# JuliaHealth/Thunderbolt.jl

Hardware: AMD Instinct MI355X
Metric: element-integrations/sec + DoF-updates/sec, 10M-hex Q1 monodomain (higher is better)
Workload: dtype f64

## Files before the change

### thunderbolt.jl_amd/csrc/tb_internal.h

```cpp
#pragma once
#include <cstdio>
#include <cstdlib>
#include <ctime>
#include <hip/hip_runtime.h>

#include <cstdint>
#include <cstdio>
#include <cstdlib>
#include <memory>
#include <string>
#include <vector>

#include "tbhip.h"
#include "tb_planners.hpp"

namespace tb {

void set_error(const char *fmt, ...);
#ifdef TB_ABLATION
inline const char *tune_env(const char *name) { return getenv(name); }
#else
inline const char *tune_env(const char *) { return nullptr; }
#endif
void set_last_kernel(const char *fmt, ...);
// ... 68 lines not shown

struct PatchPlan : plan::PatchHost {
    int version = 0;
    int64_t *d_elem_ptr = nullptr;
    int64_t *d_row_ptr = nullptr;
    int32_t *d_elem_cell = nullptr;
    uint16_t *d_elem_lrow = nullptr;
    int32_t *d_row_dof = nullptr;
};

struct PatchMatPlan {
    int version = 0;
    int max_lds_entries = 0;
    RowDesc *d_row_desc = nullptr;
    uint16_t *d_elem_rowoff = nullptr;
    uint8_t *d_colpos8 = nullptr;
    uint16_t *d_colpos16 = nullptr;
};

struct PatchFusedPlan {
    int version = 0;
    int max_lds_entries = 0, max_nodes = 0;
    int64_t nsig = 0;
    int64_t *d_node_ptr = nullptr;
    int32_t *d_pnode = nullptr;
    uint16_t *d_elem_ln = nullptr;
    uint32_t *d_elem_sig = nullptr;
    uint8_t *d_sigtab = nullptr;
    RowDesc *d_row_desc = nullptr;
    uint32_t *d_hdr = nullptr;
    double *d_pcoord = nullptr;
    uint8_t *d_rec = nullptr;
    int rec_stride = 0, rec_rm = 0, rec_nm = 0, rec_ne = 0;
};

struct VecPatchPlan {
    bool halo = false;
    int64_t n_patches = 0, total_elems = 0, total_nodes = 0;
    int max_nodes = 0, max_elems = 0;
    uint32_t *d_hdr = nullptr;
    uint16_t *d_elem_ln = nullptr;
    int32_t *d_elem_cell = nullptr;
    double *d_pcoord = nullptr;
    int32_t *d_pdof = nullptr;
};

constexpr int RED_SLOTS = 64, RED_STRIDE = 16, RED_GROUP = RED_SLOTS * RED_STRIDE;

}

struct tb_pattern;
struct tb_device {
    int id = 0;
    hipStream_t stream = nullptr;
    bool own_stream = true;
    int n_cu = 0;
    size_t hbm_bytes = 0;
    std::string name;
    tb::Status *d_status = nullptr;
    tb::Status *h_status = nullptr;
    bool defer_status = false;
    void *d_scratch = nullptr;
    size_t scratch_bytes = 0;
    double *d_slots = nullptr;
    double *d_readback = nullptr;
    double *d_tslot = nullptr;
// ... 259 lines not shown
```

### thunderbolt.jl_amd/csrc/tb_patch_fused.hip

```cpp
#include <hip/hip_runtime.h>

#include <algorithm>
#include <cstdio>
#include <cstring>
#include <vector>

#include "tb_elem.hpp"
#include "tb_forms.hpp"
#include "tb_hex8_sumfac.hpp"
#include "tb_internal.h"

namespace tb {
using namespace tbk;

struct FusedView {
    const int64_t *elem_ptr, *row_ptr, *node_ptr;
    const int32_t *elem_cell;
    const uint16_t *elem_ln;
    const uint32_t *elem_sig;
    const uint8_t *sigtab;
    const int32_t *pnode;
    const RowDesc *row_desc;
    int kcap, max_rows, max_nodes;
#ifdef TB_ABLATION
    long long *prof;
#endif
};

template <bool WK, bool WM, bool FK, bool FM, bool DIAG = false, bool ISO = false, class Meta>
__device__ __forceinline__ void hex8_instance(const double (&x)[8][3], Meta &&meta, int64_t cell, const FormArgs &faK,
                                              const FormArgs &faM, double *accK, double *accM, Status *st, const int32_t *elem_cell, int64_t e)
{
    double G[8][6], dq[8];
    if constexpr (FK) {
        const double *gp = faK.gtab + cell * 56;
#pragma unroll
        for (int q = 0; q < 8; ++q) {
#pragma unroll
            for (int k = 0; k < 6; ++k) G[q][k] = gp[7 * q + k];
            dq[q] = gp[7 * q + 6];
        }
    } else {
        auto Dq = [&](int, double(&D)[6]) { D[0] = faK.D[0]; D[1] = faK.D[1]; D[2] = faK.D[2]; D[3] = faK.D[4]; D[4] = faK.D[5]; D[5] = faK.D[8]; };
#ifdef TB_ABLATION
        if (faK.debug & 4) {
#pragma unroll
            for (int q = 0; q < 8; ++q) { dq[q] = x[q][0] + x[q][1] + x[q][2]; for (int k = 0; k < 6; ++k) G[q][k] = dq[q]; }
        } else
#endif
        if (!hex8_sf_geometry<WK, false, DIAG, ISO>(x, Dq, G, dq, ISO ? faK.iso_scale : -0.25)) { st->neg_detj = 1; st->cell = elem_cell ? elem_cell[e] : -1; }
    }
    Hex8SFK c;
    if constexpr (WK) hex8_sf_contract(G, c);
    uint4 cp[4];
    uint32_t ro[8];
    meta(cp, ro);
    bool own[8];
#pragma unroll
    for (int i = 0; i < 8; ++i) own[i] = ro[i] != 0xFFFFFFFFu;
#ifdef TB_ABLATION
    if (faK.debug & 1) {
#pragma unroll
        for (int i = 1; i < 8; ++i) own[i] = false;
        own[0] = own[0] && (G[0][0] + dq[0] == 1.2345);
    }
#endif
    auto pos = [&](int i, int j) -> uint32_t {
        const uint4 &c4 = cp[i >> 1];
        const uint32_t w = (i & 1) ? (j < 4 ? c4.z : c4.w) : (j < 4 ? c4.x : c4.y);
        return (w >> (8 * (j & 3))) & 0xffu;
    };
    if constexpr (WK) {
#pragma unroll
        for (int i = 0; i < 8; ++i)
#pragma unroll
            for (int j = i; j < 8; ++j) {
                const double v = hex8_sf_entry(c, i, j);
                if (own[i]) unsafeAtomicAdd(accK + (ro[i] + pos(i, j)), v);
                if (j > i && own[j]) unsafeAtomicAdd(accK + (ro[j] + pos(j, i)), v);
            }
    }
    if constexpr (WM) {
        if constexpr (FM) {
            double rn[8];
#pragma unroll
            for (int a = 0; a < 8; ++a) rn[a] = faM.field[cell * 8 + a];
#pragma unroll
            for (int q = 0; q < 8; ++q) {
                double r = 0.0;
#pragma unroll
                for (int a = 0; a < 8; ++a) r += Hex8<2>::N(q, a) * rn[a];
                dq[q] *= r;
            }
        } else {
#pragma unroll
            for (int q = 0; q < 8; ++q) dq[q] *= faM.rho;
        }
        double Z[3][3][3];
        hex8_sf_mass(dq, Z);
#pragma unroll
        for (int i = 0; i < 8; ++i)
            if (own[i]) {
#pragma unroll
                for (int j = 0; j < 8; ++j) unsafeAtomicAdd(accM + (ro[i] + pos(i, j)), Z[SF::ty(i, j, 0)][SF::ty(i, j, 1)][SF::ty(i, j, 2)]);
            }
    }
}

__global__ void __launch_bounds__(256)
k_tabulate_g_hex8(MeshView m, const double *__restrict__ dtab, double *__restrict__ gtab, Status *st)
{
    const int64_t cell = (int64_t)blockIdx.x * blockDim.x + threadIdx.x;
    if (cell >= m.n_cells) return;
    double x[8][3];
#pragma unroll
    for (int a = 0; a < 8; ++a) {
        const double *px = m.xyz + 3 * (int64_t)m.conn[cell * 8 + a];
        x[a][0] = px[0]; x[a][1] = px[1]; x[a][2] = px[2];
    }
    double G[8][6], dq[8];
    auto Dq = [&](int q, double(&D)[6]) {
        const double *dp = dtab + (cell * 8 + q) * 6;
#pragma unroll
        for (int k = 0; k < 6; ++k) D[k] = dp[k];
    };
    if (!hex8_sf_geometry<true, false>(x, Dq, G, dq)) { st->neg_detj = 1; st->cell = cell; }
    double *gp = gtab + cell * 56;
#pragma unroll
    for (int q = 0; q < 8; ++q) {
#pragma unroll
        for (int k = 0; k < 6; ++k) gp[7 * q + k] = G[q][k];
        gp[7 * q + 6] = dq[q];
    }
}

template <bool WK, bool WM, bool FK, bool FM>
__global__ void __launch_bounds__(256, 2)
// ... 156 lines not shown
    for (int s0 = half; s0 < nrows; s0 += 4 * (T / 32)) {
        uint4 d[4];
#pragma unroll
        for (int u = 0; u < 4; ++u) { const int s = s0 + u * (T / 32); d[u] = ((const uint4 *)desc)[s < nrows ? s : s0]; if (s >= nrows) d[u].w = 0; }
        double vK[4], vM[4];
#pragma unroll
        for (int u = 0; u < 4; ++u) {
            const uint32_t a_ = d[u].z + (hl < d[u].w ? hl : 0);
            if constexpr (WK) vK[u] = accK[a_];
            if constexpr (WM) vM[u] = accM[a_];
        }
#pragma unroll
        for (int u = 0; u < 4; ++u)
            if (hl < d[u].w) {
                const int64_t g0 = (int64_t)(((uint64_t)d[u].y << 32) | d[u].x) + hl;
                if constexpr (WK) nzK[g0] = vK[u];
                if constexpr (WM) nzM[g0] = vM[u];
            }
#pragma unroll
        for (int u = 0; u < 4; ++u)
            for (uint32_t k = hl + 32; k < d[u].w; k += 32) {
                const int64_t g0 = (int64_t)(((uint64_t)d[u].y << 32) | d[u].x) + k;
                if constexpr (WK) nzK[g0] = accK[d[u].z + k];
                if constexpr (WM) nzM[g0] = accM[d[u].z + k];
            }
    }
    TB_ST(5);
#ifdef TB_ABLATION
    if (pv.prof) { __builtin_amdgcn_s_waitcnt(0); TB_ST(6); }
#endif
#undef TB_ST
}

template <bool WK, bool WM, bool DIAG, bool ISO, int RPH, int KOFF = 0, bool WQ = true>
__global__ void __launch_bounds__(256, 2)
k_patch_hex8_record(FormArgs faK, FormArgs faM, const uint8_t *__restrict__ rec, int stride, int nem, int rm, int nm, int kcap, const uint8_t *__restrict__ sigtab, const int32_t *__restrict__ elem_cell, int pf, int prio, int stagger,
                    double *__restrict__ nzK, double *__restrict__ nzM, Status *st
#ifdef TB_ABLATION
                    , long long *prof
#endif
)
{
    extern __shared__ double lds[];
    constexpr int T = 256;
    const int tid = threadIdx.x;
    const int wave_s = __builtin_amdgcn_readfirstlane(threadIdx.x >> 6);
#ifdef TB_ABLATION
#define TB_ST(k) do { if (prof && tid == 0 && (blockIdx.x & 1023) == 7) prof[(blockIdx.x >> 10) * 8 + (k)] = wall_clock64(); } while (0)
#else
#define TB_ST(k) do { } while (0)
#endif
    TB_ST(0);
    bool slot0 = false;
    if (prio >= 2) slot0 = (__builtin_amdgcn_s_getreg((31 << 11) | 6) & 0xfffu) == 0u;
    if (prio == 1 || prio == 2) __builtin_amdgcn_s_setprio(3);
    if (stagger > 0 && blockIdx.x >= 256 && blockIdx.x < 512)
        for (int k = 0; k < stagger; k += 100) __builtin_amdgcn_s_sleep(100);
    const uint8_t *r = rec + (size_t)blockIdx.x * (size_t)stride;
    const uint4 h4 = *(const uint4 *)r;
    const uint32_t hw = h4.x;
    (void)pf;
    uint4 lnv = ((const uint4 *)(r + 16))[tid];
    const uint32_t sig = ((const uint32_t *)(r + 16 + (size_t)nem * 16))[tid];
    const uint8_t *rdp = r + 16 + (size_t)nem * 20;
    const double *pc = (const double *)(rdp + (size_t)rm * 16);
    constexpr int NX = ISO ? 6 : 5;
    uint4 rd = make_uint4(0, 0, 0, 0);
    double xc[NX];
    if (tid < rm) rd = ((const uint4 *)rdp)[tid];
    if constexpr (ISO) {
#pragma unroll
        for (int j = 0; j < 2; ++j)
#pragma unroll
            for (int d = 0; d < 3; ++d) xc[3 * j + d] = tid + j * T < nm ? pc[3 * (tid + j * T) + d] : 0.0;
    } else {
#pragma unroll
        for (int j = 0; j < NX; ++j) xc[j] = tid + j * T < 3 * nm ? pc[tid + j * T] : 0.0;
    }
    const int kblk = KOFF > 0 ? KOFF : kcap;
    double *accK = lds;
    double *accM = lds + (WK && WM ? kblk : 0);
    RowDesc *desc = (RowDesc *)(lds + (WK && WM ? 2 : 1) * kblk);
    double *xs = (double *)(desc + rm);
    {
        double2 *z = (double2 *)lds;
        const int n2 = ((WK && WM ? 2 : 1) * kblk) >> 1;
        for (int k = tid; k < n2; k += T) z[k] = make_double2(0.0, 0.0);
    }
    if (tid < rm) ((uint4 *)desc)[tid] = rd;
    if constexpr (ISO) {
        const double *Li = faK.Linv;
        auto put = [&](int node, double x0, double x1, double x2) {
            xs[3 * node] = Li[0] * x0 + Li[1] * x1 + Li[2] * x2; xs[3 * node + 1] = Li[3] * x0 + Li[4] * x1 + Li[5] * x2; xs[3 * node + 2] = Li[6] * x0 + Li[7] * x1 + Li[8] * x2;
        };
#pragma unroll
        for (int j = 0; j < 2; ++j) if (tid + j * T < nm) put(tid + j * T, xc[3 * j], xc[3 * j + 1], xc[3 * j + 2]);
        for (int k = tid + 2 * T; k < nm; k += T) put(k, pc[3 * k], pc[3 * k + 1], pc[3 * k + 2]);
    } else {
#pragma unroll
        for (int j = 0; j < NX; ++j) if (tid + j * T < 3 * nm) xs[tid + j * T] = xc[j];
        for (int k = tid + NX * T; k < 3 * nm; k += T) xs[k] = pc[k];
    }
    uint4 cp[4];
    {
        const uint4 *cpp = (const uint4 *)(sigtab + (size_t)sig * 64);
#pragma unroll
        for (int k = 0; k < 4; ++k) cp[k] = cpp[k];
    }
    const int nrows = (int)(hw & 0x3ff), ne = (int)(hw >> 21);
    TB_ST(1);
    __syncthreads();
    TB_ST(2);
    if (prio == 1) __builtin_amdgcn_s_setprio(0);
    else if (prio >= 2) { if (!slot0) __builtin_amdgcn_s_setprio(0); else if (prio == 4) __builtin_amdgcn_s_setprio(1); else __builtin_amdgcn_s_setprio(3); }
    for (int ei = tid; ei < ne; ei += T) {
        if (ei >= T) {
            lnv = ((const uint4 *)(r + 16))[ei];
            const uint4 *cpp = (const uint4 *)(sigtab + (size_t)((const uint32_t *)(r + 16 + (size_t)nem * 16))[ei] * 64);
#pragma unroll
            for (int k = 0; k < 4; ++k) cp[k] = cpp[k];
        }
        const uint32_t ln[8] = {lnv.x & 0xffffu, lnv.x >> 16, lnv.y & 0xffffu, lnv.y >> 16, lnv.z & 0xffffu, lnv.z >> 16, lnv.w & 0xffffu, lnv.w >> 16};
        double x[8][3];
#pragma unroll
        for (int a = 0; a < 8; ++a) {
            const double *px = xs + 3 * ln[a];
            x[a][0] = px[0]; x[a][1] = px[1]; x[a][2] = px[2];
        }
        uint32_t ro[8];
#pragma unroll
        for (int i = 0; i < 8; ++i) ro[i] = ln[i] < (uint32_t)nrows ? desc[ln[i]].off : 0xFFFFFFFFu;
        hex8_instance<WK, WM, false, false, DIAG, ISO>(x, [&](uint4(&c4)[4], uint32_t(&r8)[8]) { for (int k = 0; k < 4; ++k) c4[k] = cp[k]; for (int k = 0; k < 8; ++k) r8[k] = ro[k]; }, 0, faK, faM, accK, accM, st,
                                                  elem_cell, (int64_t)h4.y + ei);
    }
    TB_ST(3);
    __syncthreads();
    TB_ST(4);
    if (prio == 1 || prio == 2) __builtin_amdgcn_s_setprio(3);
    const int tidw = (int)__builtin_amdgcn_mbcnt_hi(~0u, __builtin_amdgcn_mbcnt_lo(~0u, 0u)) + 64 * wave_s;
    if constexpr (WQ) {
        const int quarter = tidw >> 4, e2 = (tidw & 15) << 1;
        constexpr int RQ = RPH / 2, RH = RQ / 2;
#pragma unroll
        for (int h = 0; h < 2; ++h) {
            uint4 d[RH];
#pragma unroll
            for (int u = 0; u < RH; ++u) { const int s = quarter + (h * RH + u) * (T / 16); d[u] = ((const uint4 *)desc)[s < nrows ? s : 0]; }
            asm volatile("" ::: "memory");
#pragma unroll
            for (int u = 0; u < RH; ++u) if (quarter + (h * RH + u) * (T / 16) >= nrows) d[u].w = 0;
            double vK[RH][2], vM[RH][2];
#pragma unroll
            for (int u = 0; u < RH; ++u) {
                const uint32_t a_ = d[u].z + ((uint32_t)e2 < d[u].w ? e2 : 0);
                if constexpr (WK) { vK[u][0] = accK[a_]; vK[u][1] = accK[a_ + 1]; }
                if constexpr (WM) { vM[u][0] = accM[a_]; vM[u][1] = accM[a_ + 1]; }
            }
#pragma unroll
            for (int u = 0; u < RH; ++u) {
                const int64_t g0 = (int64_t)(((uint64_t)d[u].y << 32) | d[u].x) + e2;
                if ((uint32_t)e2 + 1 < d[u].w) {
                    if constexpr (WK) *(double2 *)(nzK + g0) = make_double2(vK[u][0], vK[u][1]);
                    if constexpr (WM) *(double2 *)(nzM + g0) = make_double2(vM[u][0], vM[u][1]);
                } else if ((uint32_t)e2 < d[u].w) {
                    if constexpr (WK) nzK[g0] = vK[u][0];
                    if constexpr (WM) nzM[g0] = vM[u][0];
// ... 133 lines not shown
                          (size_t)2 * KOFF * sizeof(double) + (size_t)pr->rec_rm * sizeof(RowDesc) + (size_t)pr->rec_nm * 3 * sizeof(double) <= 80 * 1024;
        const size_t ldsr = (size_t)nreg * (fixm ? KOFF : pv.kcap) * sizeof(double) + (size_t)pr->rec_rm * sizeof(RowDesc) + (size_t)pr->rec_nm * 3 * sizeof(double);
        if (ldsr <= 80 * 1024) {
            constexpr int RPH = 20;
            static const bool iso_on = !(getenv("TB_PATCH_ISO") && atoi(getenv("TB_PATCH_ISO")) == 0);
            bool iso = false;
            FormArgs aMi = aM;
            if (fK && iso_on) {
                const double *D = aK.D;
                double L[3][3] = {{0, 0, 0}, {0, 0, 0}, {0, 0, 0}};
                bool pd = D[1] == D[3] && D[2] == D[6] && D[5] == D[7];
                for (int i = 0; i < 3 && pd; ++i)
                    for (int j = 0; j <= i; ++j) {
                        double sum = D[3 * i + j];
                        for (int k2 = 0; k2 < j; ++k2) sum -= L[i][k2] * L[j][k2];
                        if (i == j) { if (!(sum > 0.0)) { pd = false; break; } L[i][i] = std::sqrt(sum); }
                        else L[i][j] = sum / L[j][j];
                    }
                if (pd) {
                    double Li[3][3] = {{0, 0, 0}, {0, 0, 0}, {0, 0, 0}};
                    for (int i = 0; i < 3; ++i) {
                        Li[i][i] = 1.0 / L[i][i];
                        for (int j = 0; j < i; ++j) { double sum = 0.0; for (int k2 = j; k2 < i; ++k2) sum -= L[i][k2] * Li[k2][j]; Li[i][j] = sum / L[i][i]; }
                    }
                    const double detL = L[0][0] * L[1][1] * L[2][2];
                    for (int i = 0; i < 3; ++i) for (int j = 0; j < 3; ++j) aK.Linv[3 * i + j] = Li[i][j];
                    aK.iso_scale = -0.25 * detL;
                    aMi.rho = aM.rho * detL;
                    iso = true;
                }
            }
            static const size_t lds_pad = tune_env("TB_PATCH_LDS_PAD") ? (size_t)atol(tune_env("TB_PATCH_LDS_PAD")) : 0;
            const size_t ldsr_ = ldsr;
            auto launch_rec = [&](auto k) -> int {
                const size_t ldsr = std::max(ldsr_, lds_pad);
                TB_HIP(hipFuncSetAttribute((const void *)k, hipFuncAttributeMaxDynamicSharedMemorySize, (int)ldsr));
#ifdef TB_ABLATION
                hipLaunchKernelGGL(k, dim3((unsigned)pp->n_patches), dim3(256), ldsr, dev->stream, aK, aMi, (const uint8_t *)pr->d_rec, pr->rec_stride, pr->rec_ne, pr->rec_rm, pr->rec_nm, pv.kcap,
                                   (const uint8_t *)pf->d_sigtab, pp->d_elem_cell, pf_ahead, wave_prio, stagger, d_nzK, d_nzM, dev->d_status, d_prof);
#else
                hipLaunchKernelGGL(k, dim3((unsigned)pp->n_patches), dim3(256), ldsr, dev->stream, aK, aMi, (const uint8_t *)pr->d_rec, pr->rec_stride, pr->rec_ne, pr->rec_rm, pr->rec_nm, pv.kcap,
                                   (const uint8_t *)pf->d_sigtab, pp->d_elem_cell, pf_ahead, wave_prio, stagger, d_nzK, d_nzM, dev->d_status);
#endif
                return TB_OK;
            };
            set_last_kernel("k_patch_hex8_record<%s,%s,RPH%d%s>", fK && fM ? "K+M" : fK ? "K" : "M", !fK ? "-" : iso ? "ISO" : diag ? "DIAG" : "GEN", RPH, fK && fM && fixm ? ",KOFF4096" : "");
            static const bool wq_off = tune_env("TB_PATCH_WQ") && atoi(tune_env("TB_PATCH_WQ")) == 0;
            if (fK && fM && fixm && iso && wq_off) rc = launch_rec(k_patch_hex8_record<true, true, false, true, RPH, KOFF, false>);
            else if (fK && fM && fixm) rc = iso ? launch_rec(k_patch_hex8_record<true, true, false, true, RPH, KOFF>) : diag ? launch_rec(k_patch_hex8_record<true, true, true, false, RPH, KOFF>) : launch_rec(k_patch_hex8_record<true, true, false, false, RPH, KOFF>);
            else if (fK && fM) rc = iso ? launch_rec(k_patch_hex8_record<true, true, false, true, RPH>) : diag ? launch_rec(k_patch_hex8_record<true, true, true, false, RPH>) : launch_rec(k_patch_hex8_record<true, true, false, false, RPH>);
            else if (fK) rc = iso ? launch_rec(k_patch_hex8_record<true, false, false, true, RPH>) : diag ? launch_rec(k_patch_hex8_record<true, false, true, false, RPH>) : launch_rec(k_patch_hex8_record<true, false, false, false, RPH>);
            else rc = launch_rec(k_patch_hex8_record<false, true, false, false, RPH>);
            if (rc) return rc;
            TB_HIP(hipGetLastError());
            goto done;
        }
    }
    {
    const MeshView mv = make_view(m);
    auto launch = [&](auto ks, auto kg) -> int {
        if (staged) {
            TB_HIP(hipFuncSetAttribute((const void *)ks, hipFuncAttributeMaxDynamicSharedMemorySize, (int)lds));
            hipLaunchKernelGGL(ks, dim3((unsigned)pp->n_patches), dim3(256), lds, dev->stream, aK, aM, pv, (const uint4 *)pf->d_hdr, pf->d_pcoord, d_nzK, d_nzM, dev->d_status);
        } else {
            TB_HIP(hipFuncSetAttribute((const void *)kg, hipFuncAttributeMaxDynamicSharedMemorySize, (int)lds));
            hipLaunchKernelGGL(kg, dim3((unsigned)pp->n_patches), dim3(pp->threads), lds, dev->stream, mv, aK, aM, pv, d_nzK, d_nzM, dev->d_status);
        }
        return TB_OK;
    };
    set_last_kernel("%s<%s,%s%s%s>", staged ? "k_patch_hex8_staged" : "k_patch_hex8", fK && fM ? "K+M" : fK ? "K" : "M", !fK ? "-" : fk ? "FIELD" : diag ? "DIAG" : "GEN", fm ? ",RHO_FIELD" : "", "");
#define TB_PL(a, b, c, d) rc = launch(k_patch_hex8_staged<a, b, c, d>, k_patch_hex8<a, b, c, d>)
#define TB_PLD(a, b, c, d) rc = launch(k_patch_hex8_staged<a, b, c, d, true>, k_patch_hex8<a, b, c, d>)
    if (fK && fM) { if (fk && fm) TB_PL(true, true, true, true); else if (fk) TB_PL(true, true, true, false); else if (fm) { if (diag) TB_PLD(true, true, false, true); else TB_PL(true, true, false, true); } else { if (diag) TB_PLD(true, true, false, false); else TB_PL(true, true, false, false); } }
    else if (fK) { if (fk) TB_PL(true, false, true, false); else if (diag) TB_PLD(true, false, false, false); else TB_PL(true, false, false, false); }
    else { if (fm) TB_PL(false, true, false, true); else TB_PL(false, true, false, false); }
#undef TB_PL
#undef TB_PLD
    if (rc) return rc;
    TB_HIP(hipGetLastError());
    }
done:
#ifdef TB_ABLATION
    if (d_prof && staged) {
        std::vector<long long> h((size_t)nprof * 8);
        TB_SYNC_STREAM(dev);
// ... 18 lines not shown
```

### thunderbolt.jl_amd/csrc/tb_planners.cpp

```cpp
#include <algorithm>
#include <parallel/algorithm>
#include <cmath>
#include <cstring>
#include <numeric>

#include "tb_planners.hpp"

namespace tb {
namespace plan {

static Outcome refused(int code) { Outcome o; o.kind = Outcome::REFUSED; o.code = code; return o; }

void dof_slots(const MeshView &m, std::vector<int64_t> &ptr, std::vector<int32_t> &src)
{
    const int64_t n = m.n_cells * m.ndpc;
    ptr.assign(m.ndofs + 1, 0);
    for (int64_t i = 0; i < n; ++i) ptr[m.cell_dofs[i] + 1]++;
    for (int64_t d = 0; d < m.ndofs; ++d) ptr[d + 1] += ptr[d];
    std::vector<int64_t> pos(ptr.begin(), ptr.end() - 1);
    src.resize(n);
    for (int64_t i = 0; i < n; ++i) src[pos[m.cell_dofs[i]]++] = (int32_t)i;
}

SlotTable slot_table(const MeshView &m)
// ... 489 lines not shown
                (long long)nsig, (long long)res.lds_need, nregions);
    plan.elem_sig.resize(pp.total_elems);
#pragma omp parallel for schedule(static)
    for (int64_t e = 0; e < pp.total_elems; ++e) plan.elem_sig[e] = cell_sig[pp.h_elem_cell[e]];
    if (pp.max_rows < 1024 && max_nodes < 2048 && pp.max_elems < 2048 && pp.total_elems < (int64_t)0x7fffffff && (int64_t)pnode.size() < (int64_t)0x7fffffff) {
        plan.hdr.resize((size_t)pp.n_patches * 4);
        for (int64_t q = 0; q < pp.n_patches; ++q) {
            uint32_t *h = &plan.hdr[4 * q];
            h[0] = (uint32_t)pp.h_elem_ptr[q]; h[1] = (uint32_t)pp.h_row_ptr[q]; h[2] = (uint32_t)node_ptr[q];
            const uint32_t ne = (uint32_t)(pp.h_elem_ptr[q + 1] - pp.h_elem_ptr[q]), nr = (uint32_t)(pp.h_row_ptr[q + 1] - pp.h_row_ptr[q]),
                           nn = (uint32_t)(node_ptr[q + 1] - node_ptr[q]);
            h[3] = nr | nn << 10 | ne << 21;
        }
        plan.pcoord.resize(pnode.size() * 3);
#pragma omp parallel for schedule(static)
        for (int64_t k = 0; k < (int64_t)pnode.size(); ++k)
            for (int d = 0; d < 3; ++d) plan.pcoord[3 * k + d] = m.xyz[3 * (int64_t)pnode[k] + d];
    }
    out = std::move(plan);
    return res;
}

Records record_layout(const PatchHost &pp, int max_nodes)
{
    Records rec;
    if (pp.max_elems > 1024 || pp.max_rows > 256) return rec;
    rec.rm = (pp.max_rows + 3) & ~3; rec.nm = (max_nodes + 3) & ~3; rec.ne = std::max(256, (pp.max_elems + 63) & ~63);
    const size_t raw = 16 + (size_t)rec.ne * 20 + (size_t)rec.rm * 16 + (size_t)rec.nm * 24, stride = (raw + 127) & ~(size_t)127;
    if (stride * (size_t)pp.n_patches > ((size_t)8 << 30)) return rec;
    rec.stride = (int)stride;
    return rec;
}

void pack_records(Records &rec, int64_t np, const uint32_t *hdr, const uint16_t *ln, const uint32_t *sig, const RowDesc *desc, const double *xyz)
{
    const size_t stride = (size_t)rec.stride, o_ln = 16, o_sig = o_ln + (size_t)rec.ne * 16, o_desc = o_sig + (size_t)rec.ne * 4, o_xyz = o_desc + (size_t)rec.rm * 16;
    rec.bytes.assign(stride * (size_t)np, 0);
#pragma omp parallel for schedule(static)
    for (int64_t q = 0; q < np; ++q) {
        uint8_t *r = &rec.bytes[stride * (size_t)q];
        const uint32_t e0 = hdr[4 * q], r0 = hdr[4 * q + 1], n0 = hdr[4 * q + 2], w = hdr[4 * q + 3];
        const uint32_t nr = w & 0x3ff, nn = (w >> 10) & 0x7ff, ne = w >> 21;
        const uint32_t h4[4] = {w, e0, 0, 0};
        memcpy(r, h4, 16);
        memcpy(r + o_ln, &ln[(size_t)e0 * 8], (size_t)ne * 16);
        memcpy(r + o_sig, &sig[e0], (size_t)ne * 4);
        memcpy(r + o_desc, &desc[r0], (size_t)nr * 16);
        memcpy(r + o_xyz, &xyz[(size_t)n0 * 3], (size_t)nn * 24);
    }
}

int vec_patch_plan(const MeshView &m, const Options &o, bool halo, VecHost &out)
{
    if (m.ndpc != 8 || m.nverts != 8 || m.ncomp != 1) { set_error("vector patch plan: needs a scalar trilinear hexahedron field"); return ERR_UNSUPPORTED; }
    StageTimer timer("ensure_vec_patch_plan", o.verbose);
    const int *tile = o.vtile;
    const int64_t nc = m.n_cells;
    Keyed keyed(nc);
    CellBuckets B;
    cell_buckets(m, B);
#pragma omp parallel for schedule(static)
    for (int64_t c = 0; c < nc; ++c) {
        uint64_t t3[3];
        for (int d = 0; d < 3; ++d) t3[d] = o.full_cut ? (uint64_t)(B.bucket[3 * c + d] / tile[d]) : balanced_tile(B.bucket[3 * c + d], B.Rv[d], tile[d], halo);
        keyed[c] = {(t3[2] << 42) | (t3[1] << 21) | t3[0], (int32_t)c};
    }
    {
        std::vector<uint64_t> keys(nc);
        for (int64_t c = 0; c < nc; ++c) keys[c] = keyed[c].first;
        __gnu_parallel::sort(keys.begin(), keys.end());
        const int64_t ntiles = std::unique(keys.begin(), keys.end()) - keys.begin();
        const int64_t vol = (int64_t)tile[0] * tile[1] * tile[2];
        const double fill = ntiles > 0 ? (double)nc / ((double)ntiles * (double)vol) : 1.0;
// ... 211 lines not shown
```

### thunderbolt.jl_amd/csrc/tb_planners.hpp

```cpp
#pragma once
#include <cstdint>
#include <cstdio>
#include <ctime>
#include <vector>

namespace tb {

void set_error(const char *fmt, ...);

struct RowDesc {
    int64_t nz0;
    uint32_t off;
    uint32_t len;
};

struct StageTimer {
    const char *name;
    double t0;
    bool on, rest;
    static double now() { timespec ts; clock_gettime(CLOCK_MONOTONIC, &ts); return (double)ts.tv_sec + 1e-9 * (double)ts.tv_nsec; }
    StageTimer(const char *n, bool enabled, bool rest_line = true) : name(n), t0(0.0), on(enabled), rest(rest_line) { if (on) t0 = now(); }
    void lap(const char *what) { if (on) { const double t = now(); fprintf(stderr, "[tbhip] plan time: %-28s %-34s %8.3f s\n", name, what, t - t0); t0 = t; } }
    ~StageTimer() { if (rest) lap("(rest)"); }
};
// ... 27 lines not shown
    int patch_tile_shrink = 0;
};

struct Outcome {
    enum Kind { OK, TOO_BIG, REFUSED } kind = OK;
    int code = 0;
    int64_t lds_need = 0;
    bool ok() const { return kind == OK; }
};

struct PatchHost {
    int cells_per_patch = 0;
    int shrink = 0;
    int64_t n_patches = 0;
    int max_elems = 0, max_rows = 0, threads = 256;
    int64_t total_elems = 0, total_rows = 0;
    std::vector<int64_t> h_elem_ptr, h_row_ptr;
    std::vector<int32_t> h_elem_cell, h_row_dof;
    std::vector<uint16_t> h_elem_lrow;
};
struct MatHost { int max_lds_entries = 0; std::vector<RowDesc> row_desc; std::vector<uint16_t> rowoff, cp16; std::vector<uint8_t> cp8; };
struct FusedHost {
    int max_lds_entries = 0, max_nodes = 0;
    int64_t nsig = 0;
    std::vector<int64_t> node_ptr;
    std::vector<int32_t> pnode;
    std::vector<uint16_t> ln;
    std::vector<uint32_t> elem_sig, hdr;
    std::vector<uint8_t> sigtab;
    std::vector<RowDesc> row_desc;
    std::vector<double> pcoord;
};
struct Records { int stride = -1, rm = 0, nm = 0, ne = 0; std::vector<uint8_t> bytes; };
struct VecHost {
    bool halo = false;
    int64_t n_patches = 0, total_elems = 0, total_nodes = 0;
    int max_nodes = 0, max_elems = 0;
    std::vector<uint32_t> hdr;
    std::vector<uint16_t> ln;
    std::vector<int32_t> ecell, pdof;
    std::vector<double> pcoord;
};
struct ColorHost { int ncolors = 0; std::vector<int64_t> offsets; std::vector<int32_t> cells; };
struct SlotTable { int w = 0; std::vector<int32_t> ell, h_done; };

void dof_slots(const MeshView &m, std::vector<int64_t> &ptr, std::vector<int32_t> &src);
SlotTable slot_table(const MeshView &m);
void tensor_order(std::vector<int32_t> &ell);
int color_cells(const MeshView &m, const int32_t *cells, int64_t n, ColorHost &out);
int patch_plan(const MeshView &m, const Options &o, int leaf, int shrink, PatchHost &out);
std::vector<RowDesc> row_descs(const PatchHost &pp, const PatternView &p, int64_t &maxlen, int64_t &max_entries);
Outcome mat_extension(const MeshView &m, const PatternView &p, const PatchHost &pp, const Options &o, MatHost &out);
Outcome fused_extension(const MeshView &m, const PatternView &p, const PatchHost &pp, const Options &o, int nregions, FusedHost &out);
Records record_layout(const PatchHost &pp, int max_nodes);
void pack_records(Records &rec, int64_t np, const uint32_t *hdr, const uint16_t *ln, const uint32_t *sig, const RowDesc *desc, const double *xyz);
int vec_patch_plan(const MeshView &m, const Options &o, bool halo, VecHost &out);
Outcome fit_mat(const MeshView &m, const PatternView &p, const Options &o, FitState &st, PatchHost &cur, bool &replaced, MatHost &mat);
Outcome fit_fused(const MeshView &m, const PatternView &p, const Options &o, int nregions, FitState &st, PatchHost &cur, bool &replaced, FusedHost &fused);

}
}
```

### thunderbolt.jl_amd/csrc/tb_plans.cpp

```cpp
#include <cstring>

#include "tb_internal.h"

namespace tb {
using namespace plan;

static MeshView view(const tb_mesh *m) { return {m->n_nodes, m->n_cells, m->ndofs, m->nverts, m->ndpc, m->ncomp, m->h_xyz.data(), m->h_conn.data(), m->h_cell_dofs.data()}; }
static PatternView view(const tb_pattern *p) { return {p->n_rows, p->h_rowptr.data(), p->h_colidx.data(), p->max_row_len}; }

static bool parse3(const char *e, int *t)
{
    int a, b, c;
    if (!e || sscanf(e, "%d,%d,%d", &a, &b, &c) != 3 || a <= 0 || b <= 0 || c <= 0) return false;
    t[0] = a; t[1] = b; t[2] = c;
    return true;
}

static Options env_options()
{
    Options o;
    const char *tile = getenv("TB_PATCH_TILE"), *cells = tune_env("TB_PATCH_CELLS");
    o.tile_set = tile != nullptr;
    o.morton = !parse3(tile, o.tile) && cells;
    if (cells && atoi(cells) > 0) o.cells = atoi(cells);
// ... 164 lines not shown
    p->patch_fused = std::make_unique<PatchFusedPlan>();
    PatchFusedPlan *d = p->patch_fused.get();
    d->version = m->patches->version;
    d->max_lds_entries = h.max_lds_entries; d->max_nodes = h.max_nodes; d->nsig = h.nsig;
    const int rc = upload_all(m->dev, h.node_ptr, &d->d_node_ptr, h.pnode, &d->d_pnode, h.ln, &d->d_elem_ln, h.elem_sig, &d->d_elem_sig, h.sigtab, &d->d_sigtab,
                              h.row_desc, &d->d_row_desc, h.hdr, &d->d_hdr, h.pcoord, &d->d_pcoord);
    if (rc) free_patch_fused_plan(p);
    return rc;
}

static int ensure_patch_records_impl(tb_pattern *p)
{
    PatchFusedPlan *f = p->patch_fused.get();
    const PatchPlan *pp = p->mesh->patches.get();
    if (!f || !pp || !f->d_hdr) return TB_ERR_UNSUPPORTED;
    if (f->d_rec) return TB_OK;
    TB_NO_CAPTURE(p->mesh->dev);
    PlanTimer timer("ensure_patch_records_impl");
    Records rec = f->rec_stride < 0 ? Records() : record_layout(*pp, f->max_nodes);
    if (rec.stride < 0) { f->rec_stride = -1; return TB_ERR_UNSUPPORTED; }
    const int64_t np = pp->n_patches;
    std::vector<uint32_t> hdr((size_t)np * 4);
    std::vector<uint16_t> ln((size_t)pp->total_elems * 8);
    std::vector<uint32_t> sig((size_t)pp->total_elems);
    std::vector<RowDesc> desc((size_t)pp->total_rows);
    TB_HIP(hipMemcpy(hdr.data(), f->d_hdr, hdr.size() * 4, hipMemcpyDeviceToHost));
    TB_HIP(hipMemcpy(ln.data(), f->d_elem_ln, ln.size() * 2, hipMemcpyDeviceToHost));
    TB_HIP(hipMemcpy(sig.data(), f->d_elem_sig, sig.size() * 4, hipMemcpyDeviceToHost));
    TB_HIP(hipMemcpy(desc.data(), f->d_row_desc, desc.size() * sizeof(RowDesc), hipMemcpyDeviceToHost));
    int64_t total_nodes = 0;
    for (int64_t q = 0; q < np; ++q) total_nodes = std::max<int64_t>(total_nodes, (int64_t)hdr[4 * q + 2] + ((hdr[4 * q + 3] >> 10) & 0x7ff));
    std::vector<double> xyz((size_t)total_nodes * 3);
    TB_HIP(hipMemcpy(xyz.data(), f->d_pcoord, xyz.size() * 8, hipMemcpyDeviceToHost));
    pack_records(rec, np, hdr.data(), ln.data(), sig.data(), desc.data(), xyz.data());
    TB_HIP(hipMalloc((void **)&f->d_rec, rec.bytes.size()));
    TB_HIP(hipMemcpy(f->d_rec, rec.bytes.data(), rec.bytes.size(), hipMemcpyHostToDevice));
    f->rec_stride = rec.stride; f->rec_rm = rec.rm; f->rec_nm = rec.nm; f->rec_ne = rec.ne;
    if (getenv("TB_PLAN_VERBOSE"))
        fprintf(stderr, "[tbhip] one-trip patch records: %lld patches x %zu B (rows <= %d, nodes <= %d), %.2f GB\n", (long long)np, (size_t)rec.stride, rec.rm, rec.nm, (double)rec.bytes.size() / 1e9);
    return TB_OK;
}

int ensure_patch_records(tb_pattern *p)
{
    const int rc = ensure_patch_records_impl(p);
    if (rc != TB_OK && rc != TB_ERR_UNSUPPORTED) {
        PatchFusedPlan *f = p->patch_fused.get();
        if (f) {
            if (f->d_rec) { (void)hipFree(f->d_rec); f->d_rec = nullptr; }
            f->rec_stride = -1;
        }
        (void)hipGetLastError();
        return TB_ERR_UNSUPPORTED;
    }
    return rc;
}

int ensure_vec_patch_plan(tb_mesh *m, bool halo)
{
    if (m->vpatches[halo]) return TB_OK;
    VecHost h;
    TB_TRY(vec_patch_plan(view(m), env_options(), halo, h));
    auto &v = m->vpatches[halo];
    v = std::make_unique<VecPatchPlan>();
    v->halo = halo; v->n_patches = h.n_patches; v->total_elems = h.total_elems; v->total_nodes = h.total_nodes; v->max_nodes = h.max_nodes; v->max_elems = h.max_elems;
    const int rc = upload_all(m->dev, h.hdr, &v->d_hdr, h.ln, &v->d_elem_ln, h.ecell, &v->d_elem_cell, h.pcoord, &v->d_pcoord, h.pdof, &v->d_pdof);
    if (rc) { hipFree(v->d_hdr); hipFree(v->d_elem_ln); hipFree(v->d_elem_cell); hipFree(v->d_pcoord); hipFree(v->d_pdof); v.reset(); }
    return rc;
}

}
```

Before: 11.61 billion.

## Split patch records into general and canonical classes with compile-time column positions

Patch records are now classified on the host: a patch whose rows all have 27 entries and whose element signatures match the structured-hex stencil is marked canonical, and records are reordered so general patches come first. Canonical patches go to a separate kernel instantiation that skips the per-element signature-table loads and computes column offsets at compile time. That instantiation accumulates with explicit workgroup-scope LDS float atomics. This is meant to remove per-element sigtab gathers and position arithmetic for the regular interior of the mesh. In exchange it adds a second kernel launch, a host classification pass with an extra sigtab download during planning, and more template instantiations.

```diff
diff --git a/thunderbolt.jl_amd/csrc/tb_internal.h b/thunderbolt.jl_amd/csrc/tb_internal.h
--- a/thunderbolt.jl_amd/csrc/tb_internal.h
+++ b/thunderbolt.jl_amd/csrc/tb_internal.h
@@ -124,6 +124,7 @@
     double *d_pcoord = nullptr;
     uint8_t *d_rec = nullptr;
     int rec_stride = 0, rec_rm = 0, rec_nm = 0, rec_ne = 0;
+    int64_t rec_general = 0, rec_canonical = 0;
 };
 
 struct VecPatchPlan {
diff --git a/thunderbolt.jl_amd/csrc/tb_patch_fused.hip b/thunderbolt.jl_amd/csrc/tb_patch_fused.hip
--- a/thunderbolt.jl_amd/csrc/tb_patch_fused.hip
+++ b/thunderbolt.jl_amd/csrc/tb_patch_fused.hip
@@ -27,7 +27,17 @@
 #endif
 };
 
-template <bool WK, bool WM, bool FK, bool FM, bool DIAG = false, bool ISO = false, class Meta>
+using lds_f64 = __attribute__((address_space(3))) double;
+__device__ constexpr int canon_pos(int i, int j)
+{
+    return 13 + (SF::bit(j, 0) - SF::bit(i, 0)) + 3 * (SF::bit(j, 1) - SF::bit(i, 1)) + 9 * (SF::bit(j, 2) - SF::bit(i, 2));
+}
+__device__ __forceinline__ void lds_add(uint32_t row, int entry, double v)
+{
+    (void)__hip_atomic_fetch_add((lds_f64 *)(uintptr_t)row + entry, v, __ATOMIC_RELAXED, __HIP_MEMORY_SCOPE_WORKGROUP);
+}
+
+template <bool WK, bool WM, bool FK, bool FM, bool DIAG = false, bool ISO = false, bool CANON = false, int MOFF = 0, class Meta>
 __device__ __forceinline__ void hex8_instance(const double (&x)[8][3], Meta &&meta, int64_t cell, const FormArgs &faK,
                                               const FormArgs &faM, double *accK, double *accM, Status *st, const int32_t *elem_cell, int64_t e)
 {
@@ -76,8 +86,13 @@
 #pragma unroll
             for (int j = i; j < 8; ++j) {
                 const double v = hex8_sf_entry(c, i, j);
-                if (own[i]) unsafeAtomicAdd(accK + (ro[i] + pos(i, j)), v);
-                if (j > i && own[j]) unsafeAtomicAdd(accK + (ro[j] + pos(j, i)), v);
+                if constexpr (CANON) {
+                    if (own[i]) lds_add(ro[i], canon_pos(i, j), v);
+                    if (j > i && own[j]) lds_add(ro[j], canon_pos(j, i), v);
+                } else {
+                    if (own[i]) unsafeAtomicAdd(accK + (ro[i] + pos(i, j)), v);
+                    if (j > i && own[j]) unsafeAtomicAdd(accK + (ro[j] + pos(j, i)), v);
+                }
             }
     }
     if constexpr (WM) {
@@ -102,7 +117,11 @@
         for (int i = 0; i < 8; ++i)
             if (own[i]) {
 #pragma unroll
-                for (int j = 0; j < 8; ++j) unsafeAtomicAdd(accM + (ro[i] + pos(i, j)), Z[SF::ty(i, j, 0)][SF::ty(i, j, 1)][SF::ty(i, j, 2)]);
+                for (int j = 0; j < 8; ++j) {
+                    const double v = Z[SF::ty(i, j, 0)][SF::ty(i, j, 1)][SF::ty(i, j, 2)];
+                    if constexpr (CANON) lds_add(ro[i], MOFF + canon_pos(i, j), v);
+                    else unsafeAtomicAdd(accM + (ro[i] + pos(i, j)), v);
+                }
             }
     }
 }
@@ -325,7 +344,7 @@
 #undef TB_ST
 }
 
-template <bool WK, bool WM, bool DIAG, bool ISO, int RPH, int KOFF = 0, bool WQ = true>
+template <bool WK, bool WM, bool DIAG, bool ISO, int RPH, int KOFF = 0, bool WQ = true, bool CANON = false>
 __global__ void __launch_bounds__(256, 2)
 k_patch_hex8_record(FormArgs faK, FormArgs faM, const uint8_t *__restrict__ rec, int stride, int nem, int rm, int nm, int kcap, const uint8_t *__restrict__ sigtab, const int32_t *__restrict__ elem_cell, int pf, int prio, int stagger,
                     double *__restrict__ nzK, double *__restrict__ nzM, Status *st
@@ -354,7 +373,9 @@
     const uint32_t hw = h4.x;
     (void)pf;
     uint4 lnv = ((const uint4 *)(r + 16))[tid];
-    const uint32_t sig = ((const uint32_t *)(r + 16 + (size_t)nem * 16))[tid];
+    static_assert(!CANON || !(WK && WM) || KOFF > 0, "the canonical pair needs the mass block at a compile-time distance");
+    uint32_t sig = 0;
+    if constexpr (!CANON) sig = ((const uint32_t *)(r + 16 + (size_t)nem * 16))[tid];
     const uint8_t *rdp = r + 16 + (size_t)nem * 20;
     const double *pc = (const double *)(rdp + (size_t)rm * 16);
     constexpr int NX = ISO ? 6 : 5;
@@ -395,7 +416,7 @@
         for (int k = tid + NX * T; k < 3 * nm; k += T) xs[k] = pc[k];
     }
     uint4 cp[4];
-    {
+    if constexpr (!CANON) {
         const uint4 *cpp = (const uint4 *)(sigtab + (size_t)sig * 64);
 #pragma unroll
         for (int k = 0; k < 4; ++k) cp[k] = cpp[k];
@@ -409,9 +430,11 @@
     for (int ei = tid; ei < ne; ei += T) {
         if (ei >= T) {
             lnv = ((const uint4 *)(r + 16))[ei];
-            const uint4 *cpp = (const uint4 *)(sigtab + (size_t)((const uint32_t *)(r + 16 + (size_t)nem * 16))[ei] * 64);
-#pragma unroll
-            for (int k = 0; k < 4; ++k) cp[k] = cpp[k];
+            if constexpr (!CANON) {
+                const uint4 *cpp = (const uint4 *)(sigtab + (size_t)((const uint32_t *)(r + 16 + (size_t)nem * 16))[ei] * 64);
+#pragma unroll
+                for (int k = 0; k < 4; ++k) cp[k] = cpp[k];
+            }
         }
         const uint32_t ln[8] = {lnv.x & 0xffffu, lnv.x >> 16, lnv.y & 0xffffu, lnv.y >> 16, lnv.z & 0xffffu, lnv.z >> 16, lnv.w & 0xffffu, lnv.w >> 16};
         double x[8][3];
@@ -423,8 +446,16 @@
         uint32_t ro[8];
 #pragma unroll
         for (int i = 0; i < 8; ++i) ro[i] = ln[i] < (uint32_t)nrows ? desc[ln[i]].off : 0xFFFFFFFFu;
-        hex8_instance<WK, WM, false, false, DIAG, ISO>(x, [&](uint4(&c4)[4], uint32_t(&r8)[8]) { for (int k = 0; k < 4; ++k) c4[k] = cp[k]; for (int k = 0; k < 8; ++k) r8[k] = ro[k]; }, 0, faK, faM, accK, accM, st,
-                                                  elem_cell, (int64_t)h4.y + ei);
+        if constexpr (CANON) {
+            const uint32_t base = (uint32_t)(uintptr_t)(lds_f64 *)lds;
+#pragma unroll
+            for (int i = 0; i < 8; ++i) if (ro[i] != 0xFFFFFFFFu) ro[i] = base + 8u * ro[i];
+            hex8_instance<WK, WM, false, false, DIAG, ISO, true, (WK && WM) ? KOFF : 0>(x, [&](uint4(&)[4], uint32_t(&r8)[8]) { for (int k = 0; k < 8; ++k) r8[k] = ro[k]; }, 0, faK, faM, accK, accM, st,
+                                                                                       elem_cell, (int64_t)h4.y + ei);
+        } else {
+            hex8_instance<WK, WM, false, false, DIAG, ISO>(x, [&](uint4(&c4)[4], uint32_t(&r8)[8]) { for (int k = 0; k < 4; ++k) c4[k] = cp[k]; for (int k = 0; k < 8; ++k) r8[k] = ro[k]; }, 0, faK, faM, accK, accM, st,
+                                                           elem_cell, (int64_t)h4.y + ei);
+        }
     }
     TB_ST(3);
     __syncthreads();
@@ -624,25 +655,39 @@
             }
             static const size_t lds_pad = tune_env("TB_PATCH_LDS_PAD") ? (size_t)atol(tune_env("TB_PATCH_LDS_PAD")) : 0;
             const size_t ldsr_ = ldsr;
-            auto launch_rec = [&](auto k) -> int {
+            static const int canon_mode = getenv("TB_PATCH_CANON") ? atoi(getenv("TB_PATCH_CANON")) : -1;
+            const bool canon = canon_mode != 0 && pr->rec_canonical > 0 && !(fK && fM && !fixm) && (canon_mode > 0 || pr->rec_canonical >= (int64_t)64 * dev->n_cu);
+            const int64_t n_gen = canon ? pr->rec_general : pp->n_patches, n_can = pp->n_patches - n_gen;
+            auto launch_one = [&](auto k, int64_t first, int64_t count) -> int {
                 const size_t ldsr = std::max(ldsr_, lds_pad);
+                const uint8_t *rec0 = (const uint8_t *)pr->d_rec + (size_t)first * (size_t)pr->rec_stride;
                 TB_HIP(hipFuncSetAttribute((const void *)k, hipFuncAttributeMaxDynamicSharedMemorySize, (int)ldsr));
 #ifdef TB_ABLATION
-                hipLaunchKernelGGL(k, dim3((unsigned)pp->n_patches), dim3(256), ldsr, dev->stream, aK, aMi, (const uint8_t *)pr->d_rec, pr->rec_stride, pr->rec_ne, pr->rec_rm, pr->rec_nm, pv.kcap,
+                hipLaunchKernelGGL(k, dim3((unsigned)count), dim3(256), ldsr, dev->stream, aK, aMi, rec0, pr->rec_stride, pr->rec_ne, pr->rec_rm, pr->rec_nm, pv.kcap,
                                    (const uint8_t *)pf->d_sigtab, pp->d_elem_cell, pf_ahead, wave_prio, stagger, d_nzK, d_nzM, dev->d_status, d_prof);
 #else
-                hipLaunchKernelGGL(k, dim3((unsigned)pp->n_patches), dim3(256), ldsr, dev->stream, aK, aMi, (const uint8_t *)pr->d_rec, pr->rec_stride, pr->rec_ne, pr->rec_rm, pr->rec_nm, pv.kcap,
+                hipLaunchKernelGGL(k, dim3((unsigned)count), dim3(256), ldsr, dev->stream, aK, aMi, rec0, pr->rec_stride, pr->rec_ne, pr->rec_rm, pr->rec_nm, pv.kcap,
                                    (const uint8_t *)pf->d_sigtab, pp->d_elem_cell, pf_ahead, wave_prio, stagger, d_nzK, d_nzM, dev->d_status);
 #endif
                 return TB_OK;
             };
-            set_last_kernel("k_patch_hex8_record<%s,%s,RPH%d%s>", fK && fM ? "K+M" : fK ? "K" : "M", !fK ? "-" : iso ? "ISO" : diag ? "DIAG" : "GEN", RPH, fK && fM && fixm ? ",KOFF4096" : "");
+            auto launch_rec = [&](auto kg, auto kc) -> int {
+                if (n_gen > 0) TB_TRY(launch_one(kg, 0, n_gen));
+                if (n_can > 0) TB_TRY(launch_one(kc, n_gen, n_can));
+                return TB_OK;
+            };
+            set_last_kernel("k_patch_hex8_record<%s,%s,RPH%d%s%s>", fK && fM ? "K+M" : fK ? "K" : "M", !fK ? "-" : iso ? "ISO" : diag ? "DIAG" : "GEN", RPH, fK && fM && fixm ? ",KOFF4096" : "",
+                            n_can > 0 ? ",CANON" : "");
             static const bool wq_off = tune_env("TB_PATCH_WQ") && atoi(tune_env("TB_PATCH_WQ")) == 0;
-            if (fK && fM && fixm && iso && wq_off) rc = launch_rec(k_patch_hex8_record<true, true, false, true, RPH, KOFF, false>);
-            else if (fK && fM && fixm) rc = iso ? launch_rec(k_patch_hex8_record<true, true, false, true, RPH, KOFF>) : diag ? launch_rec(k_patch_hex8_record<true, true, true, false, RPH, KOFF>) : launch_rec(k_patch_hex8_record<true, true, false, false, RPH, KOFF>);
-            else if (fK && fM) rc = iso ? launch_rec(k_patch_hex8_record<true, true, false, true, RPH>) : diag ? launch_rec(k_patch_hex8_record<true, true, true, false, RPH>) : launch_rec(k_patch_hex8_record<true, true, false, false, RPH>);
-            else if (fK) rc = iso ? launch_rec(k_patch_hex8_record<true, false, false, true, RPH>) : diag ? launch_rec(k_patch_hex8_record<true, false, true, false, RPH>) : launch_rec(k_patch_hex8_record<true, false, false, false, RPH>);
-            else rc = launch_rec(k_patch_hex8_record<false, true, false, false, RPH>);
+#define TB_REC(wk, wm, dg, is, koff) launch_rec(k_patch_hex8_record<wk, wm, dg, is, RPH, koff>, k_patch_hex8_record<wk, wm, dg, is, RPH, koff, true, true>)
+#define TB_REC0(wk, wm, dg, is) launch_rec(k_patch_hex8_record<wk, wm, dg, is, RPH>, k_patch_hex8_record<wk, wm, dg, is, RPH>)
+            if (fK && fM && fixm && iso && wq_off) rc = launch_rec(k_patch_hex8_record<true, true, false, true, RPH, KOFF, false>, k_patch_hex8_record<true, true, false, true, RPH, KOFF, false, true>);
+            else if (fK && fM && fixm) rc = iso ? TB_REC(true, true, false, true, KOFF) : diag ? TB_REC(true, true, true, false, KOFF) : TB_REC(true, true, false, false, KOFF);
+            else if (fK && fM) rc = iso ? TB_REC0(true, true, false, true) : diag ? TB_REC0(true, true, true, false) : TB_REC0(true, true, false, false);
+            else if (fK) rc = iso ? TB_REC(true, false, false, true, 0) : diag ? TB_REC(true, false, true, false, 0) : TB_REC(true, false, false, false, 0);
+            else rc = TB_REC(false, true, false, false, 0);
+#undef TB_REC
+#undef TB_REC0
             if (rc) return rc;
             TB_HIP(hipGetLastError());
             goto done;
diff --git a/thunderbolt.jl_amd/csrc/tb_planners.cpp b/thunderbolt.jl_amd/csrc/tb_planners.cpp
--- a/thunderbolt.jl_amd/csrc/tb_planners.cpp
+++ b/thunderbolt.jl_amd/csrc/tb_planners.cpp
@@ -545,13 +545,47 @@
     return rec;
 }
 
-void pack_records(Records &rec, int64_t np, const uint32_t *hdr, const uint16_t *ln, const uint32_t *sig, const RowDesc *desc, const double *xyz)
+static inline int canonical_pos(int i, int j)
+{
+    static const int bit[3][8] = {{0, 1, 1, 0, 0, 1, 1, 0}, {0, 0, 1, 1, 0, 0, 1, 1}, {0, 0, 0, 0, 1, 1, 1, 1}};
+    return 13 + (bit[0][j] - bit[0][i]) + 3 * (bit[1][j] - bit[1][i]) + 9 * (bit[2][j] - bit[2][i]);
+}
+
+RecordClasses classify_records(int64_t np, const uint32_t *hdr, const uint16_t *ln, const uint32_t *sig, const RowDesc *desc, const uint8_t *sigtab)
+{
+    std::vector<uint8_t> canon((size_t)np, 0);
+#pragma omp parallel for schedule(static)
+    for (int64_t q = 0; q < np; ++q) {
+        const uint32_t e0 = hdr[4 * q], r0 = hdr[4 * q + 1], w = hdr[4 * q + 3];
+        const uint32_t nr = w & 0x3ff, ne = w >> 21;
+        bool ok = ne <= 256;
+        for (uint32_t k = 0; k < nr && ok; ++k) ok = desc[(size_t)r0 + k].len == 27;
+        for (uint32_t e = 0; e < ne && ok; ++e) {
+            const uint8_t *sg = sigtab + (size_t)sig[(size_t)e0 + e] * 64;
+            for (int i = 0; i < 8 && ok; ++i) {
+                if (ln[((size_t)e0 + e) * 8 + i] >= nr) continue;
+                for (int j = 0; j < 8; ++j) ok = ok && sg[i * 8 + j] == canonical_pos(i, j);
+            }
+        }
+        canon[q] = ok;
+    }
+    RecordClasses rc;
+    rc.order.reserve((size_t)np);
+    for (int64_t q = 0; q < np; ++q) if (!canon[q]) rc.order.push_back(q);
+    rc.n_general = (int64_t)rc.order.size();
+    for (int64_t q = 0; q < np; ++q) if (canon[q]) rc.order.push_back(q);
+    rc.n_canonical = np - rc.n_general;
+    return rc;
+}
+
+void pack_records(Records &rec, int64_t np, const uint32_t *hdr, const uint16_t *ln, const uint32_t *sig, const RowDesc *desc, const double *xyz, const int64_t *order)
 {
     const size_t stride = (size_t)rec.stride, o_ln = 16, o_sig = o_ln + (size_t)rec.ne * 16, o_desc = o_sig + (size_t)rec.ne * 4, o_xyz = o_desc + (size_t)rec.rm * 16;
     rec.bytes.assign(stride * (size_t)np, 0);
 #pragma omp parallel for schedule(static)
-    for (int64_t q = 0; q < np; ++q) {
-        uint8_t *r = &rec.bytes[stride * (size_t)q];
+    for (int64_t s = 0; s < np; ++s) {
+        const int64_t q = order ? order[s] : s;
+        uint8_t *r = &rec.bytes[stride * (size_t)s];
         const uint32_t e0 = hdr[4 * q], r0 = hdr[4 * q + 1], n0 = hdr[4 * q + 2], w = hdr[4 * q + 3];
         const uint32_t nr = w & 0x3ff, nn = (w >> 10) & 0x7ff, ne = w >> 21;
         const uint32_t h4[4] = {w, e0, 0, 0};
diff --git a/thunderbolt.jl_amd/csrc/tb_planners.hpp b/thunderbolt.jl_amd/csrc/tb_planners.hpp
--- a/thunderbolt.jl_amd/csrc/tb_planners.hpp
+++ b/thunderbolt.jl_amd/csrc/tb_planners.hpp
@@ -83,6 +83,7 @@
     std::vector<double> pcoord;
 };
 struct Records { int stride = -1, rm = 0, nm = 0, ne = 0; std::vector<uint8_t> bytes; };
+struct RecordClasses { int64_t n_general = 0, n_canonical = 0; std::vector<int64_t> order; };
 struct VecHost {
     bool halo = false;
     int64_t n_patches = 0, total_elems = 0, total_nodes = 0;
@@ -104,7 +105,8 @@
 Outcome mat_extension(const MeshView &m, const PatternView &p, const PatchHost &pp, const Options &o, MatHost &out);
 Outcome fused_extension(const MeshView &m, const PatternView &p, const PatchHost &pp, const Options &o, int nregions, FusedHost &out);
 Records record_layout(const PatchHost &pp, int max_nodes);
-void pack_records(Records &rec, int64_t np, const uint32_t *hdr, const uint16_t *ln, const uint32_t *sig, const RowDesc *desc, const double *xyz);
+RecordClasses classify_records(int64_t np, const uint32_t *hdr, const uint16_t *ln, const uint32_t *sig, const RowDesc *desc, const uint8_t *sigtab);
+void pack_records(Records &rec, int64_t np, const uint32_t *hdr, const uint16_t *ln, const uint32_t *sig, const RowDesc *desc, const double *xyz, const int64_t *order = nullptr);
 int vec_patch_plan(const MeshView &m, const Options &o, bool halo, VecHost &out);
 Outcome fit_mat(const MeshView &m, const PatternView &p, const Options &o, FitState &st, PatchHost &cur, bool &replaced, MatHost &mat);
 Outcome fit_fused(const MeshView &m, const PatternView &p, const Options &o, int nregions, FitState &st, PatchHost &cur, bool &replaced, FusedHost &fused);
diff --git a/thunderbolt.jl_amd/csrc/tb_plans.cpp b/thunderbolt.jl_amd/csrc/tb_plans.cpp
--- a/thunderbolt.jl_amd/csrc/tb_plans.cpp
+++ b/thunderbolt.jl_amd/csrc/tb_plans.cpp
@@ -220,12 +220,17 @@
     for (int64_t q = 0; q < np; ++q) total_nodes = std::max<int64_t>(total_nodes, (int64_t)hdr[4 * q + 2] + ((hdr[4 * q + 3] >> 10) & 0x7ff));
     std::vector<double> xyz((size_t)total_nodes * 3);
     TB_HIP(hipMemcpy(xyz.data(), f->d_pcoord, xyz.size() * 8, hipMemcpyDeviceToHost));
-    pack_records(rec, np, hdr.data(), ln.data(), sig.data(), desc.data(), xyz.data());
+    std::vector<uint8_t> sigtab((size_t)f->nsig * 64);
+    TB_HIP(hipMemcpy(sigtab.data(), f->d_sigtab, sigtab.size(), hipMemcpyDeviceToHost));
+    const RecordClasses cls = classify_records(np, hdr.data(), ln.data(), sig.data(), desc.data(), sigtab.data());
+    pack_records(rec, np, hdr.data(), ln.data(), sig.data(), desc.data(), xyz.data(), cls.order.data());
     TB_HIP(hipMalloc((void **)&f->d_rec, rec.bytes.size()));
     TB_HIP(hipMemcpy(f->d_rec, rec.bytes.data(), rec.bytes.size(), hipMemcpyHostToDevice));
     f->rec_stride = rec.stride; f->rec_rm = rec.rm; f->rec_nm = rec.nm; f->rec_ne = rec.ne;
+    f->rec_general = cls.n_general; f->rec_canonical = cls.n_canonical;
     if (getenv("TB_PLAN_VERBOSE"))
-        fprintf(stderr, "[tbhip] one-trip patch records: %lld patches x %zu B (rows <= %d, nodes <= %d), %.2f GB\n", (long long)np, (size_t)rec.stride, rec.rm, rec.nm, (double)rec.bytes.size() / 1e9);
+        fprintf(stderr, "[tbhip] one-trip patch records: %lld patches x %zu B (rows <= %d, nodes <= %d), %.2f GB; %lld general, %lld canonical\n", (long long)np, (size_t)rec.stride, rec.rm, rec.nm,
+                (double)rec.bytes.size() / 1e9, (long long)cls.n_general, (long long)cls.n_canonical);
     return TB_OK;
 }
 
```

New measurement: 11.79 billion, median of 6. 1.02x the previous value.
